# marvinli00/genie2

Measured on AMD Instinct MI355X. Metric: denoise-steps/sec (N=256, T=1000, batch=8), higher is better.
Workload: dtype f32 (pair-stack products as 3 f16 MFMAs on 2xf16-split operands, f32 accumulate); 1 GPU; unconditional N=256, T=1000, batch=8 per GPU, random-init base Denoiser (15.7M params), scale=0.6, reverse-loop steps 995..676; parallelism=replica per GPU x1, no data-path collective

## Files before the change

genie2_amd/csrc/pair_hx_kernels.hip:

```cpp
#include "hx_pair.h"


template <int NW>
__global__ __launch_bounds__(NW * 64, NW == 8 ? 1 : 2) void k_pair_transition_hx(
    float* __restrict__ z, const float* __restrict__ rmask, const unsigned char* __restrict__ wimg,
    const float* __restrict__ b1s, const float* __restrict__ b2s, int N, long long M, int n_hb, float sx, float c1, float c2, int rev) {
    extern __shared__ __attribute__((aligned(16))) unsigned char smb[];
    float* sb1 = reinterpret_cast<float*>(smb + 2 * HX_STAGE_BYTES);
    const int lane = threadIdx.x & 63, wave = UNI(threadIdx.x >> 6);
    const int h = lane >> 5, pl = lane & 31;
    const int n_wt = (int)((M + 31) / 32);
    const int n_tiles = (n_wt + NW - 1) / NW;
    const rsrc_t rw = hx_rsrc(wimg, (unsigned)(n_hb * HX_STAGE_BYTES));
    const rsrc_t rz = hx_rsrc(z, (unsigned)(M * 512));
    const rsrc_t rnull = hx_rsrc(z, 0u);
    const int lane16 = lane * 16;
    constexpr int PW = 32 / NW;
    auto issue = [&](int hb, int buf) {
#pragma unroll
        for (int q = 0; q < PW; ++q) {
            const int p = PW * wave + q;
            hx_dma(rw, smb + buf * HX_STAGE_BYTES + p * 1024, lane16, hb * HX_STAGE_BYTES + p * 1024);
        }
    };
    unsigned char* zt = smb + 2 * HX_STAGE_BYTES + 2048 + wave * HX_ZT_BYTES;
    auto tile_geom = [&](int tile, int& soff, int& nv) {
        const long long r0 = (long long)min(HX_PHYS(tile) * NW + wave, n_wt - 1) * 32;
        nv = (int)min((long long)32, M - r0);
        soff = (int)(r0 * 512);
    };
    const bool prefetch = n_hb >= 2;
    const int hq0 = max(0, n_hb / 2 - 2), hq1 = min(n_hb - 1, hq0 + 4);
    int tile = blockIdx.x;
    issue(0, 0);
    for (int u = threadIdx.x; u < n_hb * 32; u += NW * 64) sb1[u] = b1s[u];
    const float cb0 = b2s[pl], cb1 = b2s[32 + pl], cb2 = b2s[64 + pl], cb3 = b2s[96 + pl];
    float4 raw[16];
    int n_soff, n_nv;
    auto load_sync = [&](int t) {
        tile_geom(t, n_soff, n_nv);
        hx_zt_dma(rz, zt, lane, n_soff, 512, n_nv, 0); hx_vm_done(); hx_zt_read(raw, zt, pl, h, 0); hx_lds_done();
        hx_zt_dma(rz, zt, lane, n_soff, 512, n_nv, 1); hx_vm_done(); hx_zt_read(raw, zt, pl, h, 1);
    };
    load_sync(tile);
    __syncthreads();
    h8 zh[8], zl[8];
    float zres[4][16];
#pragma unroll 1
    for (; tile < n_tiles; tile += gridDim.x) {
        const int wt_raw = HX_PHYS(tile) * NW + wave;
        const bool act = wt_raw < n_wt;
        const long long row0 = (long long)(act ? wt_raw : n_wt - 1) * 32;
        const int nrows = (int)min((long long)32, M - row0);
        const bool more = tile + (int)gridDim.x < n_tiles;
        float m_own = 0.f;
        if (pl < nrows) {
            const long long idx = row0 + pl;
            const int bb = (int)(idx / ((long long)N * N));
            const int rem = (int)(idx - (long long)bb * N * N);
            m_own = rmask[bb * N + rem / N] * rmask[bb * N + rem % N];
        }
        hx_norm_split(zh, zl, raw, sx);
        f32x16 o[4];
        {
            float e0 = cb0, e1 = cb1, e2 = cb2, e3 = cb3;
            asm volatile("" : "+v"(e0), "+v"(e1), "+v"(e2), "+v"(e3));
#pragma unroll
            for (int r = 0; r < 16; ++r) { o[0][r] = e0; o[1][r] = e1; o[2][r] = e2; o[3][r] = e3; }
        }
        const rsrc_t rzz = act ? rz : rnull;
        const int voff = (4 * h * 128 + pl) * 4;
        const int srow0 = (int)(row0 * 512);
        auto stage_body = [&](int hb, auto last_tag) {
            constexpr bool LAST = decltype(last_tag)::value;
            if (more && prefetch) {
                if (hb == hq0) { tile_geom(tile + gridDim.x, n_soff, n_nv); hx_zt_dma(rz, zt, lane, n_soff, 512, n_nv, 0); }
                if (hb == hq1) { hx_zt_read(raw, zt, pl, h, 0); hx_lds_done(); hx_zt_dma(rz, zt, lane, n_soff, 512, n_nv, 1); }
            }
            if (!LAST) issue(hb + 1, (hb + 1) & 1);
            else if (more) issue(0, 0);
            const unsigned char* stage = smb + (hb & 1) * HX_STAGE_BYTES;
            f32x16 d;
#pragma unroll
            for (int r = 0; r < 16; ++r) d[r] = sb1[hb * 32 + acc_row(r, lane)];
            {
                h8 wh = hx_frag(stage, 0, 0, lane), wl = hx_frag(stage, 0, 1, lane);
#pragma unroll
                for (int kc = 0; kc < 8; ++kc) {
                    const h8 nh = hx_frag(stage, min(kc + 1, 7), 0, lane), nl = hx_frag(stage, min(kc + 1, 7), 1, lane);
                    PIPE_FENCE();
                    MFH3(wh, wl, zh[kc], zl[kc], d);
                    PIPE_FENCE();
                    wh = nh; wl = nl;
                }
            }
            if (LAST) {
#pragma unroll
                for (int r = 0; r < 8; ++r) {
                    const int so = srow0 + ((r & 3) + 8 * (r >> 2)) * 512;
                    zres[0][r] = hx_load(rzz, voff, so); zres[1][r] = hx_load(rzz, voff, so + 128);
                    zres[2][r] = hx_load(rzz, voff, so + 256); zres[3][r] = hx_load(rzz, voff, so + 384);
                }
            }
            h8 ah[2], al[2];
#pragma unroll
            for (int c = 0; c < 2; ++c) {
                float x[8];
#pragma unroll
                for (int e = 0; e < 8; ++e) x[e] = fmaxf(d[8 * c + e], 0.f);
                hx_split8(x, c1, ah[c], al[c]);
            }
            {
                h8 bh = hx_frag(stage, 8, 0, lane), bl = hx_frag(stage, 8, 1, lane);
#pragma unroll
                for (int u = 0; u < 8; ++u) {
                    const h8 nh = hx_frag(stage, 8 + min(u + 1, 7), 0, lane), nl = hx_frag(stage, 8 + min(u + 1, 7), 1, lane);
                    PIPE_FENCE();
                    MFH3(ah[u >> 2], al[u >> 2], bh, bl, o[u & 3]);
                    PIPE_FENCE();
                    bh = nh; bl = nl;
                }
            }
            __syncthreads();
        };
#pragma unroll 1
        for (int hb = 0; hb + 1 < n_hb; ++hb) stage_body(hb, std::false_type{});
        stage_body(n_hb - 1, std::true_type{});
#pragma unroll
        for (int r = 8; r < 16; ++r) {
            const int so = srow0 + ((r & 3) + 8 * (r >> 2)) * 512;
            zres[0][r] = hx_load(rzz, voff, so); zres[1][r] = hx_load(rzz, voff, so + 128);
            zres[2][r] = hx_load(rzz, voff, so + 256); zres[3][r] = hx_load(rzz, voff, so + 384);
        }
#pragma unroll
        for (int r = 0; r < 16; ++r) {
            const int rc = (r & 3) + 8 * (r >> 2);
            const float m = __shfl(m_own, rc + 4 * h);
            const int so = srow0 + rc * 512;
            const float v0 = o[0][r], v1 = o[1][r], v2 = o[2][r], v3 = o[3][r];
            hx_store(rzz, fmaf(v0, c2, zres[0][r]) * m, voff, so);
            hx_store(rzz, fmaf(v1, c2, zres[1][r]) * m, voff, so + 128);
            hx_store(rzz, fmaf(v2, c2, zres[2][r]) * m, voff, so + 256);
            hx_store(rzz, fmaf(v3, c2, zres[3][r]) * m, voff, so + 384);
        }
        if (more) {
            if (prefetch) hx_zt_read(raw, zt, pl, h, 1);
            else load_sync(tile + gridDim.x);
        }
    }
}

template <bool OUTGOING, int NW>
__global__ __launch_bounds__(NW * 64, NW == 8 ? 1 : 2) void k_trimul_proj_hx(
    const float* __restrict__ z, const float* __restrict__ rmask, const unsigned char* __restrict__ wimg,
    const float* __restrict__ bias, unsigned* __restrict__ acm, unsigned* __restrict__ bcm, int N, int NP, int n_wtiles,
    unsigned cm_bytes, unsigned z_bytes, float sx, float cpa, float cpb, float cg, int rev) {
    extern __shared__ __attribute__((aligned(16))) unsigned char smb[];
    float* sbias = reinterpret_cast<float*>(smb + 2 * HX_STAGE_BYTES);
    const int lane = threadIdx.x & 63, wave = UNI(threadIdx.x >> 6);
    const int h = lane >> 5, pl = lane & 31;
    const int ntile = (N + 31) >> 5;
    const int n_tiles = (n_wtiles + NW - 1) / NW;
    const rsrc_t rw = hx_rsrc(wimg, 8 * HX_STAGE_BYTES);
    const rsrc_t ra = hx_rsrc(acm, cm_bytes), rb = hx_rsrc(bcm, cm_bytes);
    const int lane16 = lane * 16;
    const int sstride = NP * NP * 4;
    constexpr int PW = 32 / NW;
    auto issue = [&](int pass, int buf) {
#pragma unroll
        for (int q = 0; q < PW; ++q) {
            const int p = PW * wave + q;
            hx_dma(rw, smb + buf * HX_STAGE_BYTES + p * 1024, lane16, pass * HX_STAGE_BYTES + p * 1024);
        }
    };
    unsigned char* zt = smb + 2 * HX_STAGE_BYTES + 2048 + wave * HX_ZT_BYTES;
    const rsrc_t rz = hx_rsrc(z, z_bytes);
    const int zstride = OUTGOING ? 512 : N * 512;
    auto tile_geom = [&](int tile, int& soff, int& nv) {
        const int wt = min(HX_PHYS(tile) * NW + wave, n_wtiles - 1);
        const int st = wt % ntile, line = (wt / ntile) % N, b = wt / (ntile * N);
        nv = min(32, N - st * 32);
        soff = OUTGOING ? ((b * N + line) * N + st * 32) * 512 : ((b * N + st * 32) * N + line) * 512;
    };
    int tile = blockIdx.x;
    issue(0, 0);
    for (int u = threadIdx.x; u < 512; u += NW * 64) sbias[u] = bias[u];
    __syncthreads();
    unsigned wst[8];
    f32x16 apA, agA, apB, agB;
#pragma unroll
    for (int r = 0; r < 16; ++r) { apB[r] = 0.f; agB[r] = 0.f; apA[r] = sbias[acc_row(r, lane)]; agA[r] = sbias[256 + acc_row(r, lane)]; }
    h8 zh[8], zl[8];
    float4 raw[16];
    int n_soff, n_nv;
    tile_geom(tile, n_soff, n_nv);
    hx_zt_dma(rz, zt, lane, n_soff, zstride, n_nv, 0); hx_vm_done(); hx_zt_read(raw, zt, pl, h, 0); hx_lds_done();
    hx_zt_dma(rz, zt, lane, n_soff, zstride, n_nv, 1); hx_vm_done(); hx_zt_read(raw, zt, pl, h, 1);
    int p_voff = 0x7FFFFFF0, p_so = 0;
    float p_pm = 0.f;
#pragma unroll 1
    for (; tile < n_tiles; tile += gridDim.x) {
        const int wt_raw = HX_PHYS(tile) * NW + wave;
        const bool act = wt_raw < n_wtiles;
        const int wt = act ? wt_raw : n_wtiles - 1;
        const int st = wt % ntile, line = (wt / ntile) % N, b = wt / (ntile * N);
        const int t0i = st * 32;
        const int nvalid = act ? min(32, N - t0i) : 0;
        const float msk = (pl < nvalid) ? rmask[b * N + line] * rmask[b * N + t0i + pl] : 0.f;
        const float ma = msk * cpa, mb = msk * cpb;
        const int voff = (pl < nvalid) ? (4 * h * NP * NP + pl) * 4 : 0x7FFFFFF0;
        const int sbase = ((b * 128 * NP + line) * NP + t0i) * 4;
        const bool more = tile + (int)gridDim.x < n_tiles;
        hx_norm_split(zh, zl, raw, sx);
#pragma unroll 1
        for (int pp = 0; pp < 4; ++pp) {
            {
                const int pass = 2 * pp;
                if (more) {
                    if (pp == 0) tile_geom(tile + gridDim.x, n_soff, n_nv);
                    if (pp == 2) { hx_zt_read(raw, zt, pl, h, 0); hx_lds_done(); }
                }
                issue(pass + 1, 1);
                const unsigned char* stage = smb;
                const rsrc_t e_rd = (pp == 0 || pp > 2) ? rb : ra;
                const int e_voff = pp == 0 ? p_voff : voff;
                const int e_so = pp == 0 ? p_so : sbase + ((pass - 1) & 3) * 32 * sstride;
                const float e_pm = pp == 0 ? p_pm : (pp > 2 ? mb : ma);
                HX_PROJ_STAGE(apA, agA, apB, agB);
                asm volatile("s_waitcnt vmcnt(16)" ::: "memory");
                if (more) {
                    if (pp == 0) hx_zt_dma(rz, zt, lane, n_soff, zstride, n_nv, 0, 0, 3);
                    else if (pp == 1) hx_zt_dma(rz, zt, lane, n_soff, zstride, n_nv, 0, 6, 2);
                    else if (pp == 2) hx_zt_dma(rz, zt, lane, n_soff, zstride, n_nv, 1, 0, 3);
                    else hx_zt_dma(rz, zt, lane, n_soff, zstride, n_nv, 1, 6, 2);
                }
                hx_stage_barrier();
            }
            {
                const int pass = 2 * pp + 1;
                if (pp < 3) issue(pass + 1, 0);
                else if (more) issue(0, 0);
                const unsigned char* stage = smb + HX_STAGE_BYTES;
                const rsrc_t e_rd = pp < 2 ? ra : rb;
                const int e_voff = voff;
                const int e_so = sbase + ((pass - 1) & 3) * 32 * sstride;
                const float e_pm = pp < 2 ? ma : mb;
                HX_PROJ_STAGE(apB, agB, apA, agA);
                asm volatile("s_waitcnt vmcnt(16)" ::: "memory");
                if (more) {
                    if (pp == 0) hx_zt_dma(rz, zt, lane, n_soff, zstride, n_nv, 0, 3, 3);
                    else if (pp == 2) hx_zt_dma(rz, zt, lane, n_soff, zstride, n_nv, 1, 3, 3);
                }
                hx_stage_barrier();
            }
        }
        p_voff = voff; p_so = sbase + 3 * 32 * sstride; p_pm = mb;
        if (more) hx_zt_read(raw, zt, pl, h, 1);
    }
    {
        const rsrc_t e_rd = rb;
        const int e_voff = p_voff, e_so = p_so;
        const float e_pm = p_pm;
        float t[16], u[16];
#pragma unroll
        for (int r = 0; r < 16; ++r) {
            HX_PROJ_PIECE_A(agB, r, t[r]);
            HX_PROJ_PIECE_B(apB, r, t[r], u[r]);
        }
        PIPE_FENCE();
#pragma unroll
        for (int r = 0; r < 16; ++r) HX_PROJ_PIECE_C_NOW(r, t[r], u[r]);
    }
}

#define CX_ROWB 48
template <int WT>
__global__ __launch_bounds__(256, 2) void k_trimul_contract_hx(const unsigned* __restrict__ acm, const unsigned* __restrict__ bcm,
                                                               float* __restrict__ xcm, int NP, int n_mat, unsigned cm_bytes, float cx, int rev) {
    constexpr int TM = 64 * WT;
    constexpr int PLANE = TM * CX_ROWB;
    extern __shared__ __attribute__((aligned(16))) unsigned char smb[];
    const int tid = threadIdx.x, lane = tid & 63;
    const int wave = UNI(tid >> 6);
    const int wm = wave >> 1, wn = wave & 1;
    const int tiles = (NP + TM - 1) / TM;
    const int T = tiles * tiles;
    const int n_tiles = T * ((n_mat + 7) / 8) * 8;
    const int nk = NP / 16;
    const rsrc_t ra = hx_rsrc(acm, cm_bytes), rb = hx_rsrc(bcm, cm_bytes), rx = hx_rsrc(xcm, cm_bytes);
    const int lr = tid >> 2, c4 = tid & 3;
    const int vload = (lr * NP + c4 * 4) * 4;
    const int slds = lr * CX_ROWB + c4 * 8;
    u32x4 rA[WT], rB[WT];

    auto decode = [&](int wl, int& mi, int& i0, int& j0) {
        const int w = rev ? n_tiles - 1 - wl : wl;
        const int grp = w / (8 * T), rem = w % (8 * T);
        const int tile = rem >> 3;
        mi = grp * 8 + (rem & 7);
        i0 = (tile / tiles) * TM;
        j0 = (tile % tiles) * TM;
    };
    auto gload = [&](int w, int kc) {
        int mi, i0, j0;
        decode(w, mi, i0, j0);
        const int mclamp = min(mi, n_mat - 1);
        const int mbase = mclamp * NP * NP * 4 + kc * 64;
#pragma unroll
        for (int u = 0; u < WT; ++u) {
            const int va = (i0 + 64 * u + lr < NP) ? vload : 0x7FFFFFF0, vb = (j0 + 64 * u + lr < NP) ? vload : 0x7FFFFFF0;
            rA[u] = __builtin_bit_cast(u32x4, __builtin_amdgcn_raw_buffer_load_b128(ra, va, mbase + (i0 + 64 * u) * NP * 4, 0));
            rB[u] = __builtin_bit_cast(u32x4, __builtin_amdgcn_raw_buffer_load_b128(rb, vb, mbase + (j0 + 64 * u) * NP * 4, 0));
        }
    };
    auto swrite = [&](int buf) {
        unsigned char* sa = smb + buf * 4 * PLANE + slds;
#pragma unroll
        for (int u = 0; u < WT; ++u) {
            uint2 ahi, alo, bhi, blo;
            ahi.x = __builtin_amdgcn_perm(rA[u].y, rA[u].x, 0x05040100u); ahi.y = __builtin_amdgcn_perm(rA[u].w, rA[u].z, 0x05040100u);
            alo.x = __builtin_amdgcn_perm(rA[u].y, rA[u].x, 0x07060302u); alo.y = __builtin_amdgcn_perm(rA[u].w, rA[u].z, 0x07060302u);
            bhi.x = __builtin_amdgcn_perm(rB[u].y, rB[u].x, 0x05040100u); bhi.y = __builtin_amdgcn_perm(rB[u].w, rB[u].z, 0x05040100u);
            blo.x = __builtin_amdgcn_perm(rB[u].y, rB[u].x, 0x07060302u); blo.y = __builtin_amdgcn_perm(rB[u].w, rB[u].z, 0x07060302u);
            *reinterpret_cast<uint2*>(sa + 64 * u * CX_ROWB) = ahi;
            *reinterpret_cast<uint2*>(sa + PLANE + 64 * u * CX_ROWB) = alo;
            *reinterpret_cast<uint2*>(sa + 2 * PLANE + 64 * u * CX_ROWB) = bhi;
            *reinterpret_cast<uint2*>(sa + 3 * PLANE + 64 * u * CX_ROWB) = blo;
        }
    };

    f32x16 acc[WT][WT];
#pragma unroll
    for (int m = 0; m < WT; ++m)
#pragma unroll
        for (int n = 0; n < WT; ++n) acc[m][n] = zero16();

    int w = blockIdx.x;
    if (w >= n_tiles) return;
    const int my_tiles = (n_tiles - 1 - w) / gridDim.x + 1;
    const int total = my_tiles * nk;
    gload(w, 0);
    swrite(0);
    __syncthreads();
    int kc = 0;
    const int foff = (lane & 31) * CX_ROWB + (lane >> 5) * 16;
    for (int it = 0; it < total; ++it) {
        const bool last_chunk = kc == nk - 1;
        const int wn_next = last_chunk ? w + gridDim.x : w;
        const int kc_next = last_chunk ? 0 : kc + 1;
        if (it + 1 < total) gload(wn_next, kc_next);
        const unsigned char* sa = smb + (it & 1) * 4 * PLANE + foff;
        h8 ah[WT], al[WT], bh[WT], bl[WT];
#pragma unroll
        for (int m = 0; m < WT; ++m) {
            ah[m] = *reinterpret_cast<const h8*>(sa + (wm * WT + m) * 32 * CX_ROWB);
            al[m] = *reinterpret_cast<const h8*>(sa + PLANE + (wm * WT + m) * 32 * CX_ROWB);
        }
#pragma unroll
        for (int n = 0; n < WT; ++n) {
            bh[n] = *reinterpret_cast<const h8*>(sa + 2 * PLANE + (wn * WT + n) * 32 * CX_ROWB);
            bl[n] = *reinterpret_cast<const h8*>(sa + 3 * PLANE + (wn * WT + n) * 32 * CX_ROWB);
        }
#pragma unroll
        for (int m = 0; m < WT; ++m)
#pragma unroll
            for (int n = 0; n < WT; ++n) MFH3(ah[m], al[m], bh[n], bl[n], acc[m][n]);
        if (last_chunk) {
            int mi, i0, j0;
            decode(w, mi, i0, j0);
            if (mi < n_mat) {
                const int vst = ((4 * (lane >> 5)) * NP + (lane & 31)) * 4;
#pragma unroll
                for (int m = 0; m < WT; ++m)
#pragma unroll
                    for (int n = 0; n < WT; ++n) {
                        const int ib = i0 + (wm * WT + m) * 32, jb = j0 + (wn * WT + n) * 32;
                        if (ib < NP && jb < NP) {
                            const int sbase = ((mi * NP + ib) * NP + jb) * 4;
#pragma unroll
                            for (int r = 0; r < 16; ++r) {
                                const float v = acc[m][n][r] * cx;
                                hx_store(rx, v, vst, sbase + ((r & 3) + 8 * (r >> 2)) * NP * 4);
                            }
                        }
                        acc[m][n] = zero16();
                    }
            }
        }
        if (it + 1 < total) swrite((it + 1) & 1);
        __syncthreads();
        w = wn_next;
        kc = kc_next;
    }
}

#define CB_ROWB 80
#define CB_PLANE (256 * CB_ROWB)
__global__ __launch_bounds__(512, 1) void k_trimul_contract_hx_big(const unsigned* __restrict__ acm, const unsigned* __restrict__ bcm,
                                                                   float* __restrict__ xcm, int NP, int n_mat, unsigned cm_bytes, float cx, int rev) {
    extern __shared__ __attribute__((aligned(16))) unsigned char smb[];
    const int tid = threadIdx.x, lane = tid & 63;
    const int wave = UNI(tid >> 6);
    const int wm = wave >> 1, wn = wave & 1;
    const int nk = NP / 32;
    const rsrc_t ra = hx_rsrc(acm, cm_bytes), rb = hx_rsrc(bcm, cm_bytes), rx = hx_rsrc(xcm, cm_bytes);
    const int gq = tid >> 3, pc = tid & 7;
    const int lr = (gq & 0x38) | ((gq & 1) << 2) | ((gq >> 1) & 3);
    u32x4 rA[2][4], rB[2][4];
    auto mat_of = [&](int w) { return rev ? n_mat - 1 - w : w; };
    auto gload = [&](int w, int kc, auto set_tag) {
        constexpr int S = decltype(set_tag)::value;
        const int mbase = mat_of(w) * NP * NP * 4 + kc * 128;
#pragma unroll
        for (int u = 0; u < 4; ++u) {
            const int row = 64 * u + lr;
            const int vo = row < NP ? (row * NP * 4 + pc * 16) : 0x7FFFFFF0;
            rA[S][u] = __builtin_bit_cast(u32x4, __builtin_amdgcn_raw_buffer_load_b128(ra, vo, mbase, 0));
            rB[S][u] = __builtin_bit_cast(u32x4, __builtin_amdgcn_raw_buffer_load_b128(rb, vo, mbase, 0));
        }
    };
    auto swrite = [&](auto set_tag) {
        constexpr int S = decltype(set_tag)::value;
        unsigned char* sa = smb + lr * CB_ROWB + pc * 8;
#pragma unroll
        for (int u = 0; u < 4; ++u) {
            uint2 ahi, alo, bhi, blo;
            ahi.x = __builtin_amdgcn_perm(rA[S][u].y, rA[S][u].x, 0x05040100u); ahi.y = __builtin_amdgcn_perm(rA[S][u].w, rA[S][u].z, 0x05040100u);
            alo.x = __builtin_amdgcn_perm(rA[S][u].y, rA[S][u].x, 0x07060302u); alo.y = __builtin_amdgcn_perm(rA[S][u].w, rA[S][u].z, 0x07060302u);
            bhi.x = __builtin_amdgcn_perm(rB[S][u].y, rB[S][u].x, 0x05040100u); bhi.y = __builtin_amdgcn_perm(rB[S][u].w, rB[S][u].z, 0x05040100u);
            blo.x = __builtin_amdgcn_perm(rB[S][u].y, rB[S][u].x, 0x07060302u); blo.y = __builtin_amdgcn_perm(rB[S][u].w, rB[S][u].z, 0x07060302u);
            *reinterpret_cast<uint2*>(sa + 64 * u * CB_ROWB) = ahi;
            *reinterpret_cast<uint2*>(sa + CB_PLANE + 64 * u * CB_ROWB) = alo;
            *reinterpret_cast<uint2*>(sa + 2 * CB_PLANE + 64 * u * CB_ROWB) = bhi;
            *reinterpret_cast<uint2*>(sa + 3 * CB_PLANE + 64 * u * CB_ROWB) = blo;
        }
    };
    f32x16 acc[2][4];
#pragma unroll
    for (int m = 0; m < 2; ++m)
#pragma unroll
        for (int n = 0; n < 4; ++n) acc[m][n] = zero16();
    int w = blockIdx.x;
    if (w >= n_mat) return;
    const int my = (n_mat - 1 - w) / gridDim.x + 1;
    const int total = my * nk;
    int lw = w, lkc = 0, issued = 0;
    auto advance = [&]() { if (lkc == nk - 1) { lw += gridDim.x; lkc = 0; } else ++lkc; };
    gload(lw, lkc, std::integral_constant<int, 0>{}); advance(); ++issued;
    if (issued < total) { gload(lw, lkc, std::integral_constant<int, 1>{}); advance(); ++issued; }
    int kc = 0;
    const int foff = (lane & 31) * CB_ROWB + (lane >> 5) * 16;
    const bool wave_live = 64 * wm < NP && 128 * wn < NP;
    auto body = [&](int it, auto set_tag) {
        const bool last_chunk = kc == nk - 1;
        swrite(set_tag);
        __syncthreads();
        if (issued < total) { gload(lw, lkc, set_tag); advance(); ++issued; }
        if (wave_live) {
#pragma unroll
            for (int c = 0; c < 2; ++c) {
                const unsigned char* sa = smb + foff + c * 32;
                h8 ah[2], al[2], bh[4], bl[4];
#pragma unroll
                for (int m = 0; m < 2; ++m) {
                    ah[m] = *reinterpret_cast<const h8*>(sa + (wm * 2 + m) * 32 * CB_ROWB);
                    al[m] = *reinterpret_cast<const h8*>(sa + CB_PLANE + (wm * 2 + m) * 32 * CB_ROWB);
                }
#pragma unroll
                for (int n = 0; n < 4; ++n) {
                    bh[n] = *reinterpret_cast<const h8*>(sa + 2 * CB_PLANE + (wn * 4 + n) * 32 * CB_ROWB);
                    bl[n] = *reinterpret_cast<const h8*>(sa + 3 * CB_PLANE + (wn * 4 + n) * 32 * CB_ROWB);
                }
#pragma unroll
                for (int m = 0; m < 2; ++m)
#pragma unroll
                    for (int n = 0; n < 4; ++n) MFH3(ah[m], al[m], bh[n], bl[n], acc[m][n]);
            }
        }
        if (last_chunk) {
            const int mi = mat_of(w);
            const int vst = ((4 * (lane >> 5)) * NP + (lane & 31)) * 4;
#pragma unroll
            for (int m = 0; m < 2; ++m)
#pragma unroll
                for (int n = 0; n < 4; ++n) {
                    const int ib = (wm * 2 + m) * 32, jb = (wn * 4 + n) * 32;
                    if (ib < NP && jb < NP) {
                        const int sbase = ((mi * NP + ib) * NP + jb) * 4;
#pragma unroll
                        for (int r = 0; r < 16; ++r) {
                            const float v = acc[m][n][r] * cx;
                            hx_store(rx, v, vst, sbase + ((r & 3) + 8 * (r >> 2)) * NP * 4);
                        }
                    }
                    acc[m][n] = zero16();
                }
            w += gridDim.x;
            kc = 0;
        } else
            ++kc;
        __syncthreads();
    };
    for (int it = 0; it < total; it += 2) {
        body(it, std::integral_constant<int, 0>{});
        if (it + 1 < total) body(it + 1, std::integral_constant<int, 1>{});
    }
}

template <int NW>
__global__ __launch_bounds__(NW * 64, NW == 8 ? 1 : 2) void k_trimul_out_hx_r(
    float* __restrict__ z, const float* __restrict__ xcm, const unsigned char* __restrict__ wimg,
    const float* __restrict__ bgs, const float* __restrict__ bzs, int N, int NP, int n_wtiles, unsigned cm_bytes,
    unsigned z_bytes, float sx, float cg, float cz, int rev) {
    extern __shared__ __attribute__((aligned(16))) unsigned char smb[];
    const int lane = threadIdx.x & 63, wave = UNI(threadIdx.x >> 6);
    const int h = lane >> 5, pl = lane & 31;
    const int ntile = (N + 31) >> 5;
    const int n_tiles = (n_wtiles + NW - 1) / NW;
    const rsrc_t rw = hx_rsrc(wimg, 4 * HX_STAGE_BYTES);
    const rsrc_t rx = hx_rsrc(xcm, cm_bytes), rz = hx_rsrc(z, z_bytes);
    const int lane16 = lane * 16;
    constexpr int PW = 32 / NW;
    auto issue = [&](int s, int buf) {
#pragma unroll
        for (int q = 0; q < PW; ++q) {
            const int p = PW * wave + q;
            hx_dma(rw, smb + buf * HX_STAGE_BYTES + p * 1024, lane16, s * HX_STAGE_BYTES + p * 1024);
        }
    };
    int tile = blockIdx.x;
    issue(0, 0); issue(1, 1); issue(2, 2); issue(3, 3);
    hx_stage_landed();
    __syncthreads();
#pragma unroll 1
    for (; tile < n_tiles; tile += gridDim.x) {
        const int wt_raw = HX_PHYS(tile) * NW + wave;
        const bool act = wt_raw < n_wtiles;
        const int wt = act ? wt_raw : n_wtiles - 1;
        const int st = wt % ntile, i = (wt / ntile) % N, b = wt / (ntile * N);
        const int t0 = st * 32;
        const int nvalid = act ? min(32, N - t0) : 0;
        const int prow0 = (b * N + i) * N + t0;
        h8 zh[8], zl[8], xh[8], xl[8];
        {
            float4 raw[16], rawz[16];
            const int cs = NP * NP * 4;
            const int vx = (8 * h * NP * NP + pl) * 4;
            const int sxo = ((b * 128 * NP + i) * NP + t0) * 4;
#pragma unroll
            for (int kc = 0; kc < 8; ++kc) {
                raw[2 * kc].x = hx_load(rx, vx, sxo + (16 * kc + 0) * cs); raw[2 * kc].y = hx_load(rx, vx, sxo + (16 * kc + 1) * cs);
                raw[2 * kc].z = hx_load(rx, vx, sxo + (16 * kc + 2) * cs); raw[2 * kc].w = hx_load(rx, vx, sxo + (16 * kc + 3) * cs);
                raw[2 * kc + 1].x = hx_load(rx, vx, sxo + (16 * kc + 4) * cs); raw[2 * kc + 1].y = hx_load(rx, vx, sxo + (16 * kc + 5) * cs);
                raw[2 * kc + 1].z = hx_load(rx, vx, sxo + (16 * kc + 6) * cs); raw[2 * kc + 1].w = hx_load(rx, vx, sxo + (16 * kc + 7) * cs);
            }
            {
                const float* zrow = z + ((size_t)(prow0 + min(pl, min(32, N - t0) - 1))) * 128 + 8 * h;
#pragma unroll
                for (int kc = 0; kc < 8; ++kc) {
                    rawz[2 * kc] = *reinterpret_cast<const float4*>(zrow + 16 * kc);
                    rawz[2 * kc + 1] = *reinterpret_cast<const float4*>(zrow + 16 * kc + 4);
                }
            }
            hx_norm_split(xh, xl, raw, sx);
            hx_norm_split(zh, zl, rawz, sx);
        }
        const int voff = (4 * h * 128 + pl) * 4;
#pragma unroll
        for (int half = 0; half < 2; ++half) {
            f32x16 ga, gb;
            {
                const unsigned char* stage = smb + (2 * half) * HX_STAGE_BYTES;
                float c0 = bgs[(2 * half) * 32 + pl], c1 = bgs[(2 * half + 1) * 32 + pl];
                asm volatile("" : "+v"(c0), "+v"(c1));
#pragma unroll
                for (int r = 0; r < 16; ++r) { ga[r] = c0; gb[r] = c1; }
                h8 f0 = hx_frag(stage, 0, 0, lane), f0l = hx_frag(stage, 0, 1, lane), f1 = hx_frag(stage, 8, 0, lane),
                   f1l = hx_frag(stage, 8, 1, lane);
#pragma unroll
                for (int kc = 0; kc < 8; ++kc) {
                    const int kn = min(kc + 1, 7);
                    const h8 n0 = hx_frag(stage, kn, 0, lane), n0l = hx_frag(stage, kn, 1, lane), n1 = hx_frag(stage, 8 + kn, 0, lane),
                             n1l = hx_frag(stage, 8 + kn, 1, lane);
                    PIPE_FENCE();
                    MFH3(zh[kc], zl[kc], f0, f0l, ga);
                    MFH3(zh[kc], zl[kc], f1, f1l, gb);
                    PIPE_FENCE();
                    f0 = n0; f0l = n0l; f1 = n1; f1l = n1l;
                }
#pragma unroll
                for (int r = 0; r < 16; ++r) {
                    ga[r] = cz * __builtin_amdgcn_rcpf(1.0f + __builtin_amdgcn_exp2f(ga[r] * cg));
                    gb[r] = cz * __builtin_amdgcn_rcpf(1.0f + __builtin_amdgcn_exp2f(gb[r] * cg));
                }
            }
            {
                const unsigned char* stage = smb + (2 * half + 1) * HX_STAGE_BYTES;
                const int ob = 2 * half;
                f32x16 a0, a1;
                float c0 = bzs[ob * 32 + pl], c1 = bzs[(ob + 1) * 32 + pl];
                asm volatile("" : "+v"(c0), "+v"(c1));
#pragma unroll
                for (int r = 0; r < 16; ++r) { a0[r] = c0; a1[r] = c1; }
                const int h4 = 4 * h;
                float zp0[16], zp1[16];
                if (half == 1) {
#pragma unroll
                    for (int r = 0; r < 16; ++r) {
                        const int rc = (r & 3) + 8 * (r >> 2);
                        const int so = (prow0 + rc) * 512 + ob * 128;
                        const int vr = (h4 < nvalid - rc) ? voff : 0x7FFFFFF0;
                        zp0[r] = hx_load(rz, vr, so);
                        zp1[r] = hx_load(rz, vr, so + 128);
                    }
                }
                h8 f0 = hx_frag(stage, 0, 0, lane), f0l = hx_frag(stage, 0, 1, lane), f1 = hx_frag(stage, 8, 0, lane),
                   f1l = hx_frag(stage, 8, 1, lane);
#pragma unroll
                for (int kc = 0; kc < 8; ++kc) {
                    const int kn = min(kc + 1, 7);
                    const h8 n0 = hx_frag(stage, kn, 0, lane), n0l = hx_frag(stage, kn, 1, lane), n1 = hx_frag(stage, 8 + kn, 0, lane),
                             n1l = hx_frag(stage, 8 + kn, 1, lane);
                    PIPE_FENCE();
                    MFH3(xh[kc], xl[kc], f0, f0l, a0);
                    MFH3(xh[kc], xl[kc], f1, f1l, a1);
                    PIPE_FENCE();
                    f0 = n0; f0l = n0l; f1 = n1; f1l = n1l;
                }
#pragma unroll
                for (int r0 = 0; r0 < 16; r0 += 8) {
                    float zr0[8], zr1[8];
                    int vo[8];
#pragma unroll
                    for (int q = 0; q < 8; ++q) {
                        const int rc = ((r0 + q) & 3) + 8 * ((r0 + q) >> 2);
                        const int so = (prow0 + rc) * 512 + ob * 128;
                        vo[q] = (h4 < nvalid - rc) ? voff : 0x7FFFFFF0;
                        if (half == 1) { zr0[q] = zp0[r0 + q]; zr1[q] = zp1[r0 + q]; }
                        else { zr0[q] = hx_load(rz, vo[q], so); zr1[q] = hx_load(rz, vo[q], so + 128); }
                    }
#pragma unroll
                    for (int q = 0; q < 8; ++q) {
                        const int rc = ((r0 + q) & 3) + 8 * ((r0 + q) >> 2);
                        const int so = (prow0 + rc) * 512 + ob * 128;
                        const float u0 = a0[r0 + q], u1 = a1[r0 + q], g0 = ga[r0 + q], g1 = gb[r0 + q];
                        hx_store(rz, fmaf(u0, g0, zr0[q]), vo[q], so);
                        hx_store(rz, fmaf(u1, g1, zr1[q]), vo[q], so + 128);
                    }
                    PIPE_FENCE();
                }
            }
        }
    }
}

static int g_hx_cu = 0;
static int hx_num_cu() {
    if (!g_hx_cu) { int dev = 0; hipDeviceProp_t pr; (void)hipGetDevice(&dev); (void)hipGetDeviceProperties(&pr, dev); g_hx_cu = pr.multiProcessorCount > 0 ? pr.multiProcessorCount : 256; }
    return g_hx_cu;
}
static int hx_nw() { return 8; }
static unsigned hx_grid(long long n_tiles, int nw) {
    const long long cap = (nw == 8 ? 1LL : 2LL) * hx_num_cu();
    return (unsigned)(n_tiles < cap ? n_tiles : cap);
}

void launch_pair_transition_hx(genie_ctx* h, hipStream_t st, const PairLayerW& w) {
    const int N = h->N;
    const long long M = (long long)h->B * N * N;
    const long long n_wt = (M + 31) / 32;
    const int n_hb = h->d.pair_transition_n * 4;
    const HxTransW& x = w.hx_pt;
    hipLaunchKernelGGL(k_pair_transition_hx<8>, dim3(hx_grid((n_wt + 7) / 8, 8)), dim3(512), HX_LDS_BYTES, st, h->p, h->rmaskf, x.img,
                       x.b1s, x.b2s, N, M, n_hb, x.sx, x.c1, x.c2, (int)(h->hx_launches++ & 1));
}

struct HxTriGeom {
    int N, NP, ntile, nw, n_wt;
    unsigned cm_bytes, z_bytes;
};
static HxTriGeom tri_geom(const genie_ctx* h) {
    HxTriGeom g;
    g.N = h->N; g.NP = h->NP; g.ntile = (g.N + 31) / 32; g.nw = hx_nw();
    g.n_wt = h->B * g.N * g.ntile;
    g.cm_bytes = (unsigned)((size_t)h->B * 128 * g.NP * g.NP * 4);
    g.z_bytes = (unsigned)((size_t)h->B * g.N * g.N * 512);
    return g;
}

static void hx_trimul_proj(genie_ctx* h, hipStream_t st, const TriMulW& w, bool outgoing) {
    const HxTriGeom g = tri_geom(h);
    const HxTriW& x = w.hx;
    unsigned* acm = reinterpret_cast<unsigned*>(h->acm);
    unsigned* bcm = reinterpret_cast<unsigned*>(h->bcm);
    ProfScope ps(h, st, KC_TRIMUL_PROJ);
    const dim3 grid(hx_grid((g.n_wt + g.nw - 1) / g.nw, g.nw)), block(g.nw * 64);
    const int rev = (int)(h->hx_launches++ & 1);
#define HX_PROJ(OUT, NWV) hipLaunchKernelGGL((k_trimul_proj_hx<OUT, NWV>), grid, block, HX_LDS_BYTES, st, h->p, h->rmaskf, x.img_proj, \
                                         x.bias_proj, acm, bcm, g.N, g.NP, g.n_wt, g.cm_bytes, g.z_bytes, x.sx, x.cpa, x.cpb, x.cg, rev)
    if (outgoing) HX_PROJ(true, 8);
    else HX_PROJ(false, 8);
#undef HX_PROJ
}

static void hx_trimul_contract(genie_ctx* h, hipStream_t st, const TriMulW& w, bool transposed) {
    const HxTriGeom g = tri_geom(h);
    const HxTriW& x = w.hx;
    ProfScope ps(h, st, KC_TRIMUL_CONTRACT);
    const int BC = h->B * h->d.c_hidden_mul;
    const int ncu = hx_num_cu();
    const int rev = (int)(h->hx_launches++ & 1);
    const unsigned* acm = reinterpret_cast<const unsigned*>(h->acm);
    const unsigned* bcm = reinterpret_cast<const unsigned*>(h->bcm);
    const unsigned* pa = transposed ? bcm : acm;
    const unsigned* pb = transposed ? acm : bcm;
    if (g.NP > 192 && g.NP <= 256) {
        hipLaunchKernelGGL(k_trimul_contract_hx_big, dim3(BC < ncu ? BC : ncu), dim3(512), 4 * CB_PLANE, st, pa, pb, h->xcm, g.NP, BC, g.cm_bytes,
                           x.cx, rev);
    } else if (g.NP >= 128) {
        const int tiles = (g.NP + 127) / 128;
        const int n_tiles = tiles * tiles * ((BC + 7) / 8) * 8;
        hipLaunchKernelGGL(k_trimul_contract_hx<2>, dim3(n_tiles < 3 * ncu ? n_tiles : 3 * ncu), dim3(256), 2 * 4 * 128 * CX_ROWB, st,
                           pa, pb, h->xcm, g.NP, BC, g.cm_bytes, x.cx, rev);
    } else {
        const int tiles = (g.NP + 63) / 64;
        const int n_tiles = tiles * tiles * ((BC + 7) / 8) * 8;
        hipLaunchKernelGGL(k_trimul_contract_hx<1>, dim3(n_tiles < 4 * ncu ? n_tiles : 4 * ncu), dim3(256), 2 * 4 * 64 * CX_ROWB, st,
                           pa, pb, h->xcm, g.NP, BC, g.cm_bytes, x.cx, rev);
    }
}

static void hx_trimul_out(genie_ctx* h, hipStream_t st, const TriMulW& w) {
    const HxTriGeom g = tri_geom(h);
    const HxTriW& x = w.hx;
    ProfScope ps(h, st, KC_TRIMUL_OUT);
    hipLaunchKernelGGL(k_trimul_out_hx_r<8>, dim3(hx_grid((g.n_wt + 7) / 8, 8)), dim3(512), 4 * HX_STAGE_BYTES, st, h->p, h->xcm,
                       x.img_out, x.bgs, x.bzs, g.N, g.NP, g.n_wt, g.cm_bytes, g.z_bytes, x.sx, x.cgo, x.cz, (int)(h->hx_launches++ & 1));
}

void launch_trimul_hx(genie_ctx* h, hipStream_t st, const TriMulW& w, bool outgoing) {
    hx_trimul_proj(h, st, w, outgoing);
    hx_trimul_contract(h, st, w, false);
    hx_trimul_out(h, st, w);
}

void launch_pair_fused(genie_ctx* h, hipStream_t st, const HxFusedW& f, const HxTriW& o, const HxTransW* t, const HxTriW* p, bool col);
bool launch_pair_stack_fused(genie_ctx* h, hipStream_t st, float* tap_trimul_out0, float* tap_layer0) {
    const int L = h->d.n_pair_transform_layer;
    if (!h->hx || L < 1 || getenv("GENIE_NO_PAIR_FUSE")) return false;
    if (h->d.n_head_tri > 0) return false;
    const size_t pbytes = (size_t)h->B * h->N * h->N * h->d.c_p * 4;
    hx_trimul_proj(h, st, h->pair[0].out, true);
    for (int l = 0; l < L; ++l) {
        const PairLayerW& W = h->pair[l];
        hx_trimul_contract(h, st, W.out, true);
        { ProfScope ps(h, st, KC_PAIR_FUSED_A); launch_pair_fused(h, st, W.fa, W.out.hx, nullptr, &W.in.hx, true); }
        if (l == 0 && tap_trimul_out0) (void)hipMemcpyAsync(tap_trimul_out0, h->p, pbytes, hipMemcpyDeviceToDevice, st);
        hx_trimul_contract(h, st, W.in, false);
        {
            ProfScope ps(h, st, KC_PAIR_FUSED_B);
            launch_pair_fused(h, st, W.fb, W.in.hx, &W.hx_pt, l + 1 < L ? &h->pair[l + 1].out.hx : nullptr, false);
        }
        if (l == 0 && tap_layer0) (void)hipMemcpyAsync(tap_layer0, h->p, pbytes, hipMemcpyDeviceToDevice, st);
    }
    return true;
}


#define IB_UNITS 24
__global__ __launch_bounds__(256) void k_ipa_bias_hx(const float* __restrict__ z, const unsigned char* __restrict__ wimg, float inv_sw,
                                                     const float* __restrict__ bias, float* __restrict__ out, int B, int N, int LH,
                                                     int n_tiles, int rev, unsigned* pmax) {
    extern __shared__ __attribute__((aligned(16))) unsigned char ibw[];
    float* sbias = reinterpret_cast<float*>(ibw + IB_UNITS * 2048);
    const int tid = threadIdx.x, lane = tid & 63, wave = tid >> 6;
    for (int u = tid; u < IB_UNITS * 128; u += 256) reinterpret_cast<uint4*>(ibw)[u] = reinterpret_cast<const uint4*>(wimg)[u];
    if (tid < 96) sbias[tid] = tid < LH ? bias[tid] : 0.f;
    __syncthreads();
    const int n = lane & 31, hf = lane >> 5;
    const int jt = (N + 31) >> 5;
    float amax = 0.f;
    for (int t = blockIdx.x * 4 + wave; t < n_tiles; t += gridDim.x * 4) {
        const int tt = rev ? n_tiles - 1 - t : t;
        const int j0 = (tt % jt) * 32;
        const int bi = tt / jt;
        const int j = min(j0 + n, N - 1);
        const float* row = z + ((size_t)bi * N + j) * 128 + 8 * hf;
        float4 x[8][2];
#pragma unroll
        for (int s = 0; s < 8; ++s) {
            x[s][0] = *reinterpret_cast<const float4*>(row + 16 * s);
            x[s][1] = *reinterpret_cast<const float4*>(row + 16 * s + 4);
        }
        float m = 0.f;
#pragma unroll
        for (int s = 0; s < 8; ++s) {
            m = fmaxf(m, fmaxf(fmaxf(fabsf(x[s][0].x), fabsf(x[s][0].y)), fmaxf(fabsf(x[s][0].z), fabsf(x[s][0].w))));
            m = fmaxf(m, fmaxf(fmaxf(fabsf(x[s][1].x), fabsf(x[s][1].y)), fmaxf(fabsf(x[s][1].z), fabsf(x[s][1].w))));
        }
        m = fmaxf(m, __shfl_xor(m, 32));
        amax = fmaxf(amax, m);
        const int e = (int)((__builtin_bit_cast(unsigned, m) >> 23) & 255u);
        const bool tiny = e < 16;
        const float sc = tiny ? 1.0f : __builtin_bit_cast(float, (unsigned)(268 - e) << 23);
        const float isc = (tiny ? 1.0f : __builtin_bit_cast(float, (unsigned)(e - 14) << 23)) * inv_sw;
        f32x16 acc[3];
#pragma unroll
        for (int blk = 0; blk < 3; ++blk)
#pragma unroll
            for (int r = 0; r < 16; ++r) acc[blk][r] = 0.f;
#pragma unroll
        for (int s = 0; s < 8; ++s) {
            const float xs[8] = {x[s][0].x, x[s][0].y, x[s][0].z, x[s][0].w, x[s][1].x, x[s][1].y, x[s][1].z, x[s][1].w};
            h8 bh, bl;
            hx_split8(xs, sc, bh, bl);
#pragma unroll
            for (int blk = 0; blk < 3; ++blk) {
                const h8 ah = hx_frag(ibw, blk * 8 + s, 0, lane), al = hx_frag(ibw, blk * 8 + s, 1, lane);
                MFH3(ah, al, bh, bl, acc[blk]);
            }
        }
        if (j0 + n < N) {
            const int b = bi / N, i = bi - b * N;
#pragma unroll
            for (int blk = 0; blk < 3; ++blk)
#pragma unroll
                for (int r = 0; r < 16; ++r) {
                    const int o = blk * 32 + (r & 3) + 8 * (r >> 2) + 4 * hf;
                    if (o < LH) out[((((size_t)o * B + b) * N + i) * N) + j0 + n] = fmaf(acc[blk][r], isc, sbias[o]);
                }
        }
    }
#pragma unroll
    for (int o = 32; o > 0; o >>= 1) amax = fmaxf(amax, __shfl_xor(amax, o));
    if (lane == 0 && __float_as_uint(amax) > *reinterpret_cast<volatile unsigned*>(pmax)) atomicMax(pmax, __float_as_uint(amax));
}

bool launch_ipa_bias_hx(genie_ctx* h, hipStream_t st) {
    const int LH = h->d.n_structure_layer * h->d.n_head_ipa;
    if (!h->hx || LH > 96) return false;
    const HxGemmW* w = nullptr;
    for (int i = 0; i < h->n_hxg; ++i)
        if (h->hxg[i].w == h->ipa_bias_w) w = &h->hxg[i];
    if (!w) return false;
    const int N = h->N, n_tiles = h->B * N * ((N + 31) / 32);
    const int grid = n_tiles / 4 < 2 * hx_num_cu() ? (n_tiles + 3) / 4 : 2 * hx_num_cu();
    (void)hipMemsetAsync(h->pmax, 0, sizeof(unsigned), st);
    hipLaunchKernelGGL(k_ipa_bias_hx, dim3(grid), dim3(256), IB_UNITS * 2048 + 96 * 4, st, h->p, w->img, w->inv_s, h->ipa_bias_b, h->ipa_bias,
                       h->B, N, LH, n_tiles, (int)(h->hx_launches & 1), h->pmax);
    return true;
}

void pair_hx_kernels_init() {
#define HX_ATTR(k) (void)hipFuncSetAttribute(reinterpret_cast<const void*>(k), hipFuncAttributeMaxDynamicSharedMemorySize, HX_LDS_BYTES)
    HX_ATTR((k_trimul_proj_hx<true, 8>)); HX_ATTR((k_trimul_proj_hx<false, 8>));
    HX_ATTR(k_trimul_out_hx_r<8>);
    (void)hipFuncSetAttribute(reinterpret_cast<const void*>(k_trimul_contract_hx_big), hipFuncAttributeMaxDynamicSharedMemorySize, 4 * CB_PLANE);
#undef HX_ATTR
    (void)hipFuncSetAttribute(reinterpret_cast<const void*>(k_pair_transition_hx<8>), hipFuncAttributeMaxDynamicSharedMemorySize, HX_LDS_BYTES);
    (void)hipFuncSetAttribute(reinterpret_cast<const void*>(k_ipa_bias_hx), hipFuncAttributeMaxDynamicSharedMemorySize, IB_UNITS * 2048 + 96 * 4);
}
```

Before: 112.3 batch-steps/s.

## Double-buffer LDS in big trimul contract and interleave fill with MFMAs

Rewrites the big triangle-multiplication contraction kernel to use two LDS buffers, so the next chunk's global loads and hi/lo-split LDS writes are interleaved piecewise with the MFMA loop on the current buffer. This removes one barrier per chunk and the serial swrite-then-compute phase. The epilogue now stages accumulator tiles through LDS and writes them out as 128-bit stores instead of scalar stores. It also drops the wave_live guard and doubles the LDS footprint, and row masking now handles only the last 64-row group. That assumes NP>192, which the launch condition guarantees.

New measurement: 111.0 batch-steps/s. 1.1% lower.

```diff
diff --git a/genie2_amd/csrc/pair_hx_kernels.hip b/genie2_amd/csrc/pair_hx_kernels.hip
--- a/genie2_amd/csrc/pair_hx_kernels.hip
+++ b/genie2_amd/csrc/pair_hx_kernels.hip
@@ -396,6 +396,8 @@
 
 #define CB_ROWB 80
 #define CB_PLANE (256 * CB_ROWB)
+#define CB_BUF (4 * CB_PLANE)
+#define CB_TROWB 144
 __global__ __launch_bounds__(512, 1) void k_trimul_contract_hx_big(const unsigned* __restrict__ acm, const unsigned* __restrict__ bcm,
                                                                    float* __restrict__ xcm, int NP, int n_mat, unsigned cm_bytes, float cx, int rev) {
     extern __shared__ __attribute__((aligned(16))) unsigned char smb[];
@@ -408,78 +410,107 @@
     const int lr = (gq & 0x38) | ((gq & 1) << 2) | ((gq >> 1) & 3);
     u32x4 rA[2][4], rB[2][4];
     auto mat_of = [&](int w) { return rev ? n_mat - 1 - w : w; };
-    auto gload = [&](int w, int kc, auto set_tag) {
-        constexpr int S = decltype(set_tag)::value;
-        const int mbase = mat_of(w) * NP * NP * 4 + kc * 128;
-#pragma unroll
-        for (int u = 0; u < 4; ++u) {
-            const int row = 64 * u + lr;
-            const int vo = row < NP ? (row * NP * 4 + pc * 16) : 0x7FFFFFF0;
-            rA[S][u] = __builtin_bit_cast(u32x4, __builtin_amdgcn_raw_buffer_load_b128(ra, vo, mbase, 0));
-            rB[S][u] = __builtin_bit_cast(u32x4, __builtin_amdgcn_raw_buffer_load_b128(rb, vo, mbase, 0));
-        }
-    };
-    auto swrite = [&](auto set_tag) {
-        constexpr int S = decltype(set_tag)::value;
-        unsigned char* sa = smb + lr * CB_ROWB + pc * 8;
-#pragma unroll
-        for (int u = 0; u < 4; ++u) {
-            uint2 ahi, alo, bhi, blo;
-            ahi.x = __builtin_amdgcn_perm(rA[S][u].y, rA[S][u].x, 0x05040100u); ahi.y = __builtin_amdgcn_perm(rA[S][u].w, rA[S][u].z, 0x05040100u);
-            alo.x = __builtin_amdgcn_perm(rA[S][u].y, rA[S][u].x, 0x07060302u); alo.y = __builtin_amdgcn_perm(rA[S][u].w, rA[S][u].z, 0x07060302u);
-            bhi.x = __builtin_amdgcn_perm(rB[S][u].y, rB[S][u].x, 0x05040100u); bhi.y = __builtin_amdgcn_perm(rB[S][u].w, rB[S][u].z, 0x05040100u);
-            blo.x = __builtin_amdgcn_perm(rB[S][u].y, rB[S][u].x, 0x07060302u); blo.y = __builtin_amdgcn_perm(rB[S][u].w, rB[S][u].z, 0x07060302u);
-            *reinterpret_cast<uint2*>(sa + 64 * u * CB_ROWB) = ahi;
-            *reinterpret_cast<uint2*>(sa + CB_PLANE + 64 * u * CB_ROWB) = alo;
-            *reinterpret_cast<uint2*>(sa + 2 * CB_PLANE + 64 * u * CB_ROWB) = bhi;
-            *reinterpret_cast<uint2*>(sa + 3 * CB_PLANE + 64 * u * CB_ROWB) = blo;
-        }
-    };
-    f32x16 acc[2][4];
-#pragma unroll
-    for (int m = 0; m < 2; ++m)
-#pragma unroll
-        for (int n = 0; n < 4; ++n) acc[m][n] = zero16();
+    const int vo_lo = lr * NP * 4 + pc * 16;
+    const int vo_hi = 192 + lr < NP ? vo_lo : 0x7FFFFFF0;
+    const int urow = 64 * NP * 4;
     int w = blockIdx.x;
     if (w >= n_mat) return;
     const int my = (n_mat - 1 - w) / gridDim.x + 1;
     const int total = my * nk;
     int lw = w, lkc = 0, issued = 0;
-    auto advance = [&]() { if (lkc == nk - 1) { lw += gridDim.x; lkc = 0; } else ++lkc; };
-    gload(lw, lkc, std::integral_constant<int, 0>{}); advance(); ++issued;
-    if (issued < total) { gload(lw, lkc, std::integral_constant<int, 1>{}); advance(); ++issued; }
+    auto req_addr = [&](int& mbase, int& v_lo, int& v_hi) {
+        const bool on = issued < total;
+        mbase = on ? mat_of(lw) * NP * NP * 4 + lkc * 128 : 0;
+        v_lo = on ? vo_lo : 0x7FFFFFF0;
+        v_hi = on ? vo_hi : 0x7FFFFFF0;
+    };
+    auto req_done = [&]() {
+        if (lkc == nk - 1) { lw += gridDim.x; lkc = 0; } else ++lkc;
+        ++issued;
+    };
+    auto gload_piece = [&](int mbase, int v_lo, int v_hi, int u, int op, auto set_tag) {
+        constexpr int S = decltype(set_tag)::value;
+        const int vo = u == 3 ? v_hi : v_lo;
+        if (op == 0) rA[S][u] = __builtin_bit_cast(u32x4, __builtin_amdgcn_raw_buffer_load_b128(ra, vo, mbase + u * urow, 0));
+        else rB[S][u] = __builtin_bit_cast(u32x4, __builtin_amdgcn_raw_buffer_load_b128(rb, vo, mbase + u * urow, 0));
+    };
+    auto fill_piece = [&](unsigned char* sf, int u, int op, auto set_tag) {
+        constexpr int S = decltype(set_tag)::value;
+        const u32x4 r = op == 0 ? rA[S][u] : rB[S][u];
+        uint2 hi, lo;
+        hi.x = __builtin_amdgcn_perm(r.y, r.x, 0x05040100u); hi.y = __builtin_amdgcn_perm(r.w, r.z, 0x05040100u);
+        lo.x = __builtin_amdgcn_perm(r.y, r.x, 0x07060302u); lo.y = __builtin_amdgcn_perm(r.w, r.z, 0x07060302u);
+        *reinterpret_cast<uint2*>(sf + (2 * op) * CB_PLANE + 64 * u * CB_ROWB) = hi;
+        *reinterpret_cast<uint2*>(sf + (2 * op + 1) * CB_PLANE + 64 * u * CB_ROWB) = lo;
+    };
+    f32x16 acc[2][4];
+#pragma unroll
+    for (int m = 0; m < 2; ++m)
+#pragma unroll
+        for (int n = 0; n < 4; ++n) acc[m][n] = zero16();
+    const int soff = lr * CB_ROWB + pc * 8;
+    const int foff = (lane & 31) * CB_ROWB + (lane >> 5) * 16;
+    {
+        int mbase, v_lo, v_hi;
+        req_addr(mbase, v_lo, v_hi);
+#pragma unroll
+        for (int q = 0; q < 8; ++q) gload_piece(mbase, v_lo, v_hi, q >> 1, q & 1, std::integral_constant<int, 0>{});
+        req_done();
+        req_addr(mbase, v_lo, v_hi);
+#pragma unroll
+        for (int q = 0; q < 8; ++q) gload_piece(mbase, v_lo, v_hi, q >> 1, q & 1, std::integral_constant<int, 1>{});
+        req_done();
+        req_addr(mbase, v_lo, v_hi);
+#pragma unroll
+        for (int q = 0; q < 8; ++q) {
+            fill_piece(smb + soff, q >> 1, q & 1, std::integral_constant<int, 0>{});
+            gload_piece(mbase, v_lo, v_hi, q >> 1, q & 1, std::integral_constant<int, 0>{});
+        }
+        req_done();
+    }
+    __syncthreads();
     int kc = 0;
-    const int foff = (lane & 31) * CB_ROWB + (lane >> 5) * 16;
-    const bool wave_live = 64 * wm < NP && 128 * wn < NP;
-    auto body = [&](int it, auto set_tag) {
+    auto body = [&](auto cur_tag) {
+        constexpr int S = decltype(cur_tag)::value, F = 1 - S;
+        const std::integral_constant<int, F> fill_tag{};
         const bool last_chunk = kc == nk - 1;
-        swrite(set_tag);
-        __syncthreads();
-        if (issued < total) { gload(lw, lkc, set_tag); advance(); ++issued; }
-        if (wave_live) {
-#pragma unroll
-            for (int c = 0; c < 2; ++c) {
-                const unsigned char* sa = smb + foff + c * 32;
-                h8 ah[2], al[2], bh[4], bl[4];
-#pragma unroll
-                for (int m = 0; m < 2; ++m) {
-                    ah[m] = *reinterpret_cast<const h8*>(sa + (wm * 2 + m) * 32 * CB_ROWB);
-                    al[m] = *reinterpret_cast<const h8*>(sa + CB_PLANE + (wm * 2 + m) * 32 * CB_ROWB);
-                }
-#pragma unroll
-                for (int n = 0; n < 4; ++n) {
-                    bh[n] = *reinterpret_cast<const h8*>(sa + 2 * CB_PLANE + (wn * 4 + n) * 32 * CB_ROWB);
-                    bl[n] = *reinterpret_cast<const h8*>(sa + 3 * CB_PLANE + (wn * 4 + n) * 32 * CB_ROWB);
-                }
-#pragma unroll
-                for (int m = 0; m < 2; ++m)
-#pragma unroll
-                    for (int n = 0; n < 4; ++n) MFH3(ah[m], al[m], bh[n], bl[n], acc[m][n]);
-            }
-        }
+        int mbase, v_lo, v_hi;
+        req_addr(mbase, v_lo, v_hi);
+        const unsigned char* sa = smb + S * CB_BUF + foff;
+        unsigned char* sf = smb + F * CB_BUF + soff;
+        h8 ah[2], al[2], bh[2], bl[2];
+        auto read_a = [&](int c) {
+#pragma unroll
+            for (int m = 0; m < 2; ++m) {
+                ah[m] = *reinterpret_cast<const h8*>(sa + c * 32 + (wm * 2 + m) * 32 * CB_ROWB);
+                al[m] = *reinterpret_cast<const h8*>(sa + c * 32 + CB_PLANE + (wm * 2 + m) * 32 * CB_ROWB);
+            }
+        };
+        auto read_b = [&](int k) {
+            const int c = k >> 2, n = k & 3;
+            bh[k & 1] = *reinterpret_cast<const h8*>(sa + c * 32 + 2 * CB_PLANE + (wn * 4 + n) * 32 * CB_ROWB);
+            bl[k & 1] = *reinterpret_cast<const h8*>(sa + c * 32 + 3 * CB_PLANE + (wn * 4 + n) * 32 * CB_ROWB);
+        };
+        read_a(0);
+        read_b(0);
+#pragma unroll
+        for (int k = 0; k < 8; ++k) {
+            if (k < 7) read_b(k + 1);
+            MFH3(ah[0], al[0], bh[k & 1], bl[k & 1], acc[0][k & 3]);
+            MFH3(ah[1], al[1], bh[k & 1], bl[k & 1], acc[1][k & 3]);
+            if (k == 3) read_a(1);
+            fill_piece(sf, k >> 1, k & 1, fill_tag);
+            gload_piece(mbase, v_lo, v_hi, k >> 1, k & 1, fill_tag);
+            PIPE_FENCE();
+        }
+        req_done();
         if (last_chunk) {
+            __syncthreads();
             const int mi = mat_of(w);
-            const int vst = ((4 * (lane >> 5)) * NP + (lane & 31)) * 4;
+            unsigned char* st = smb + S * CB_BUF + wave * (32 * CB_TROWB);
+            float* stw = reinterpret_cast<float*>(st + (4 * (lane >> 5)) * CB_TROWB) + (lane & 31);
+            const unsigned char* str = st + (lane >> 3) * CB_TROWB + (lane & 7) * 16;
+            const int vst = ((lane >> 3) * NP + (lane & 7) * 4) * 4;
 #pragma unroll
             for (int m = 0; m < 2; ++m)
 #pragma unroll
@@ -488,10 +519,14 @@
                     if (ib < NP && jb < NP) {
                         const int sbase = ((mi * NP + ib) * NP + jb) * 4;
 #pragma unroll
-                        for (int r = 0; r < 16; ++r) {
-                            const float v = acc[m][n][r] * cx;
-                            hx_store(rx, v, vst, sbase + ((r & 3) + 8 * (r >> 2)) * NP * 4);
-                        }
+                        for (int r = 0; r < 16; ++r) stw[((r & 3) + 8 * (r >> 2)) * (CB_TROWB / 4)] = acc[m][n][r] * cx;
+                        asm volatile("" ::: "memory");
+                        u32x4 v[4];
+#pragma unroll
+                        for (int q = 0; q < 4; ++q) v[q] = *reinterpret_cast<const u32x4*>(str + 8 * q * CB_TROWB);
+                        asm volatile("" ::: "memory");
+#pragma unroll
+                        for (int q = 0; q < 4; ++q) __builtin_amdgcn_raw_buffer_store_b128(v[q], rx, vst, sbase + 8 * q * NP * 4, 0);
                     }
                     acc[m][n] = zero16();
                 }
@@ -502,8 +537,8 @@
         __syncthreads();
     };
     for (int it = 0; it < total; it += 2) {
-        body(it, std::integral_constant<int, 0>{});
-        if (it + 1 < total) body(it + 1, std::integral_constant<int, 1>{});
+        body(std::integral_constant<int, 0>{});
+        body(std::integral_constant<int, 1>{});
     }
 }
 
@@ -715,7 +750,7 @@
     const unsigned* pa = transposed ? bcm : acm;
     const unsigned* pb = transposed ? acm : bcm;
     if (g.NP > 192 && g.NP <= 256) {
-        hipLaunchKernelGGL(k_trimul_contract_hx_big, dim3(BC < ncu ? BC : ncu), dim3(512), 4 * CB_PLANE, st, pa, pb, h->xcm, g.NP, BC, g.cm_bytes,
+        hipLaunchKernelGGL(k_trimul_contract_hx_big, dim3(BC < ncu ? BC : ncu), dim3(512), 2 * CB_BUF, st, pa, pb, h->xcm, g.NP, BC, g.cm_bytes,
                            x.cx, rev);
     } else if (g.NP >= 128) {
         const int tiles = (g.NP + 127) / 128;
@@ -855,7 +890,7 @@
 #define HX_ATTR(k) (void)hipFuncSetAttribute(reinterpret_cast<const void*>(k), hipFuncAttributeMaxDynamicSharedMemorySize, HX_LDS_BYTES)
     HX_ATTR((k_trimul_proj_hx<true, 8>)); HX_ATTR((k_trimul_proj_hx<false, 8>));
     HX_ATTR(k_trimul_out_hx_r<8>);
-    (void)hipFuncSetAttribute(reinterpret_cast<const void*>(k_trimul_contract_hx_big), hipFuncAttributeMaxDynamicSharedMemorySize, 4 * CB_PLANE);
+    (void)hipFuncSetAttribute(reinterpret_cast<const void*>(k_trimul_contract_hx_big), hipFuncAttributeMaxDynamicSharedMemorySize, 2 * CB_BUF);
 #undef HX_ATTR
     (void)hipFuncSetAttribute(reinterpret_cast<const void*>(k_pair_transition_hx<8>), hipFuncAttributeMaxDynamicSharedMemorySize, HX_LDS_BYTES);
     (void)hipFuncSetAttribute(reinterpret_cast<const void*>(k_ipa_bias_hx), hipFuncAttributeMaxDynamicSharedMemorySize, IB_UNITS * 2048 + 96 * 4);
```
